# dernasherbrezon/sdr-server

Measured on AMD Instinct MI355X. Metric: input IQ Msamples/s processed (all clients), 2.016 Msps->48 kHz xlating FIR, higher is better.
Workload: dtype f32; 1 GPU; 1024 clients x 48 kHz off one 2.016 Msps cu8 stream, D=42, 505 taps, 262144-byte blocks (BASELINE configs[3]; N=1: the >=1000-client single-GPU target); clients_total=1024, clients_per_gpu=1024, blocks_per_call=8, mode=optimized, parallelism=single GPU, rccl_ranks=1, feed=xlating_multi (C host)

## Files before the change

sdr-server_amd/csrc/xl_dev_inline.h:

```cpp
#ifndef XL_DEV_INLINE_H_
#define XL_DEV_INLINE_H_
#include "xl_device.h"
#include "xl_q15_narrow.h"

typedef float v2f __attribute__((ext_vector_type(2)));
typedef float v4f __attribute__((ext_vector_type(4)));
typedef const float __attribute__((address_space(4))) *cfloat_p;
typedef const uint32_t __attribute__((address_space(4))) *cu32_p;

#define XL_DEV static __device__ __forceinline__
#define XL_MEM __device__ __forceinline__

XL_DEV v2f xl_sample(const void *__restrict__ p, int fmt, uint32_t i) {
  v2f r;
  if (fmt == XLF_CU8) {
    const uint32_t v = reinterpret_cast<const uint16_t *>(p)[i];
    r.x = ((float)(v & 0xFFu) - 127.5f) / 128.0f;
    r.y = ((float)(v >> 8) - 127.5f) / 128.0f;
  } else if (fmt == XLF_CS8) {
    const int32_t v = reinterpret_cast<const int16_t *>(p)[i];
    r.x = (float)((int32_t)(int8_t)(v & 0xFF)) / 128.0f;
    r.y = (float)(v >> 8) / 128.0f;
  } else if (fmt == XLF_CS16) {
    const int32_t v = reinterpret_cast<const int32_t *>(p)[i];
// ... 72 lines not shown
};

template <int MODE>
XL_DEV v2f xl_rotate(const v2f a, const v2f p) {
  v2f r;
  if (MODE == 0) {
    r.x = a.x * p.x - a.y * p.y;
    r.y = a.x * p.y + a.y * p.x;
  } else {
    r.x = __builtin_fmaf(-a.y, p.y, a.x * p.x);
    r.y = __builtin_fmaf(a.y, p.x, a.x * p.y);
  }
  return r;
}

XL_DEV void xl_nco_step(v2f &p, const v2f inc) {
  v2f t1, t2;
  asm volatile(
      "v_pk_mul_f32 %0, %2, %3 op_sel_hi:[1,0]\n\t"
      "v_pk_mul_f32 %1, %2, %3 op_sel:[0,1] op_sel_hi:[1,1]"
      : "=&v"(t1), "=&v"(t2)
      : "v"(p), "v"(inc));
  asm volatile("v_pk_add_f32 %0, %1, %2 op_sel:[0,1] op_sel_hi:[1,0] neg_lo:[0,1]" : "=v"(p) : "v"(t1), "v"(t2));
}

XL_DEV v2f xl_nco_next(const v2f p, const v2f inc) {
  v2f t1, t2, r;
  asm volatile(
      "v_pk_mul_f32 %0, %3, %4 op_sel_hi:[1,0]\n\t"
      "v_pk_mul_f32 %1, %3, %4 op_sel:[0,1] op_sel_hi:[1,1]\n\t"
      "v_pk_add_f32 %2, %0, %1 op_sel:[0,1] op_sel_hi:[1,0] neg_lo:[0,1]"
      : "=&v"(t1), "=&v"(t2), "=&v"(r)
      : "v"(p), "v"(inc));
  return r;
}

XL_DEV v2f xl_nco_next_fma(const v2f p, const v2f inc) {
  v2f t, r;
  asm volatile(
      "v_pk_mul_f32 %0, %2, %3 op_sel:[1,1] op_sel_hi:[1,0]\n\t"
      "v_pk_fma_f32 %1, %2, %3, %0 op_sel_hi:[0,1,1] neg_lo:[0,0,1]"
      : "=&v"(t), "=&v"(r)
      : "v"(p), "v"(inc));
  return r;
}
XL_DEV v2f xl_nco_next_any(const v2f p, const v2f inc, const uint32_t flags) {
  return (flags & XL_POS_FMA_STEP) ? xl_nco_next_fma(p, inc) : xl_nco_next(p, inc);
}

XL_DEV v2f xl_nco_role_step(const v2f p, const v2f inc, const uint32_t flags) {
  float a, b, c, d;
  if (flags & XL_POS_FMA_STEP) {
    asm volatile(
        "v_mul_f32 %0, %3, %5\n\t"
        "v_mul_f32 %1, %3, %4\n\t"
        "v_fma_f32 %0, %2, %4, -%0\n\t"
        "v_fma_f32 %1, %2, %5, %1"
        : "=&v"(a), "=&v"(b)
        : "v"(p.x), "v"(p.y), "v"(inc.x), "v"(inc.y));
    return (v2f){a, b};
  }
  asm volatile(
      "v_mul_f32 %0, %4, %6\n\t"
      "v_mul_f32 %1, %5, %7\n\t"
      "v_mul_f32 %2, %4, %7\n\t"
      "v_mul_f32 %3, %5, %6\n\t"
      "v_sub_f32 %0, %0, %1\n\t"
      "v_add_f32 %1, %3, %2"
      : "=&v"(a), "=&v"(b), "=&v"(c), "=&v"(d)
      : "v"(p.x), "v"(p.y), "v"(inc.x), "v"(inc.y));
  return (v2f){a, b};
}

XL_DEV v2f xl_nco_renorm(const v2f p) {
  const double mag2 = (double)p.x * (double)p.x + (double)p.y * (double)p.y;
  const float mag = (float)__dsqrt_rn(mag2);
  return (v2f){p.x / mag, p.y / mag};
}

template <bool PACKED>
XL_DEV void xl_nco_client_chain(const XlNcoClient k, const XlBnd bnd, const uint32_t kb, const uint32_t ke,
                                const float2 *state_src, float2 *state_dst, float2 *__restrict__ tab,
                                unsigned long long *stamp = nullptr) {
  v2f p = {state_src[k.slot].x, state_src[k.slot].y};
  if (stamp) {
    asm volatile("s_waitcnt vmcnt(0)" ::: "memory");
    stamp[0] = wall_clock64();
  }
  if (bnd.K == 0u) {
    state_dst[k.slot] = make_float2(p.x, p.y);
    return;
  }
  const v2f inc = {k.incr.x, k.incr.y};
  v2f *__restrict__ o = reinterpret_cast<v2f *>(tab) + (k.out_off >> XL_PH_SHIFT);
  v4f *__restrict__ o4 = reinterpret_cast<v4f *>(o);
  uint32_t m = kb;
  while (m < ke) {
    const uint32_t nb = xl_bnd_next(bnd, m);
    const uint32_t me = nb < ke ? nb : ke;
    for (; m < me && (m & (2u * XL_PH_STRIDE - 1u)) != 0u; ++m) {
      if (tab != nullptr && (m & (XL_PH_STRIDE - 1u)) == 0u) o[m >> XL_PH_SHIFT] = p;
      p = PACKED ? xl_nco_next_any(p, inc, bnd.flags) : xl_nco_role_step(p, inc, bnd.flags);
    }
    for (; !(bnd.flags & XL_POS_FMA_STEP) && m + 2u * XL_PH_STRIDE <= me; m += 2u * XL_PH_STRIDE) {
      const v2f q0 = p;
      for (uint32_t i = 0; i < XL_PH_STRIDE; i += 16u) {
#pragma unroll
        for (int j = 0; j < 16; ++j) p = PACKED ? xl_nco_next(p, inc) : xl_nco_role_step(p, inc, 0u);
      }
      const v2f q1 = p;
      for (uint32_t i = 0; i < XL_PH_STRIDE; i += 16u) {
#pragma unroll
        for (int j = 0; j < 16; ++j) p = PACKED ? xl_nco_next(p, inc) : xl_nco_role_step(p, inc, 0u);
      }
      if (tab != nullptr) o4[m >> (XL_PH_SHIFT + 1u)] = (v4f){q0.x, q0.y, q1.x, q1.y};
    }
    for (; m < me; ++m) {
      if (tab != nullptr && (m & (XL_PH_STRIDE - 1u)) == 0u) o[m >> XL_PH_SHIFT] = p;
      p = PACKED ? xl_nco_next_any(p, inc, bnd.flags) : xl_nco_role_step(p, inc, bnd.flags);
    }
    if (me == nb) p = xl_nco_renorm(p);
  }
  if (stamp) stamp[1] = wall_clock64();
  state_dst[k.slot] = make_float2(p.x, p.y);
}

XL_DEV XlBnd xl_nco_bnd(const XlNcoClient k, const XlPos pos, const uint32_t explicit_K) {
  XlBnd b;
  if (explicit_K != 0xFFFFFFFFu) {
    b.j0 = 0u, b.D = k.D, b.S = 0xFFFFFFFFu, b.G = 1u, b.K = explicit_K;
  } else {
    const XlDyn d = xl_grid_dyn(k.D, 1u, k.rem0, 0u, pos);
    b.j0 = d.j0, b.D = k.D, b.S = pos.S, b.G = pos.G, b.K = d.K;
  }
  b.flags = pos.pad;
  return b;
}

template <class Store>
XL_DEV void xl_phase_walk(v2f p, const uint32_t m0, const uint32_t count, const v2f inc, const XlBnd bnd, Store store) {
  uint32_t m = m0 & ~(XL_PH_STRIDE - 1u);
  uint32_t nb = xl_bnd_next(bnd, m);
  const uint32_t end = m0 + count;
  for (; m < end; ++m) {
    if (m >= m0) store(m - m0, p);
    p = xl_nco_next_any(p, inc, bnd.flags);
    if (m + 1u == nb) {
      p = xl_nco_renorm(p);
      nb = xl_bnd_next(bnd, m + 1u);
    }
  }
}

#endif
```

sdr-server_amd/csrc/xl_grid.h:

```cpp
#ifndef XL_GRID_H_
#define XL_GRID_H_
#include <stdint.h>

#define XL_HCAP 16384u
#define XL_PH_STRIDE 16u
#define XL_PH_SHIFT 4u

#if defined(__HIPCC__)
#define XL_HD __host__ __device__ static inline
#else
#define XL_HD static inline
#endif

typedef struct XlPos {
  uint32_t trel;
  uint32_t S;
  uint32_t G;
  uint32_t pad;
} XlPos;
#define XL_POS_NORENORM 1u
#define XL_POS_FMA_STEP 2u

typedef struct XlDyn {
  uint32_t base;
  uint32_t K;
  uint32_t zero_below;
  uint32_t j0;
} XlDyn;

XL_HD XlDyn xl_grid_dyn_cap(uint32_t D, uint32_t T, uint32_t rem0, uint32_t hv0, XlPos p, uint32_t hcap) {
  const uint32_t rem = (rem0 % D + p.trel % D) % D;
  const uint32_t j0 = (D - rem) % D;
  const uint32_t N = p.S * p.G;
  uint32_t hv = hv0 + (p.trel < hcap ? p.trel : hcap);
  XlDyn d;
  if (hv > hcap) hv = hcap;
  d.j0 = j0;
  d.K = N > j0 ? (N - j0 + D - 1u) / D : 0u;
  d.base = hcap - (T - 1u) + j0;
  d.zero_below = hcap - hv;
  return d;
}

XL_HD XlDyn xl_grid_dyn(uint32_t D, uint32_t T, uint32_t rem0, uint32_t hv0, XlPos p) {
  return xl_grid_dyn_cap(D, T, rem0, hv0, p, XL_HCAP);
}

XL_HD XlPos xl_grid_next(XlPos p) {
  XlPos n = p;
  n.trel = p.trel + p.S * p.G;
  return n;
}

XL_HD uint32_t xl_grid_mstart(uint32_t j0, uint32_t D, uint32_t S, uint32_t g) {
  const uint32_t n = g * S;
  return n > j0 ? (n - j0 + D - 1u) / D : 0u;
}

typedef struct XlBnd {
  uint32_t j0, D, S, G, K;
  uint32_t flags;
} XlBnd;

XL_HD uint32_t xl_bnd_next(const XlBnd b, uint32_t m) {
  uint32_t g, nb;
  if (b.flags & XL_POS_NORENORM) return 0xFFFFFFFFu;
  if (b.G <= 1u) return b.K;
  g = (b.j0 + m * b.D) / b.S;
  if (g + 1u >= b.G) return b.K;
  nb = xl_grid_mstart(b.j0, b.D, b.S, g + 1u);
  return nb < b.K ? nb : b.K;
}

XL_HD uint32_t xl_merge_j0(uint32_t j0_ref, uint32_t delta, uint32_t D) {
  const uint32_t j = j0_ref + delta;
  return j >= D ? j - D : j;
}
XL_HD uint32_t xl_merge_shift(uint32_t j0_ref, uint32_t delta, uint32_t D) { return j0_ref + delta >= D ? 0u : 1u; }
XL_HD uint32_t xl_merge_points(uint32_t D, XlPos p) { return (p.S * p.G + D - 1u) / D + 1u; }
XL_HD uint32_t xl_merge_outputs(uint32_t j0_ref, uint32_t delta, uint32_t D, XlPos p) {
  const uint32_t N = p.S * p.G, Ka = N / D;
  return Ka + (xl_merge_j0(j0_ref, delta, D) < N - Ka * D ? 1u : 0u);
}

typedef struct XlColDuty {
  XlBnd bnd;
  uint32_t shift;
  uint32_t ibeg;
  uint32_t m0;
  uint32_t ok;
  uint32_t tab;
} XlColDuty;
XL_HD XlColDuty xl_col_duty(uint32_t j0_ref, uint32_t delta, uint32_t D, XlPos p, uint32_t V, uint32_t s, uint32_t g, int vacant) {
  XlColDuty d;
  uint32_t q0;
  d.bnd.j0 = xl_merge_j0(j0_ref, delta, D), d.bnd.D = D, d.bnd.S = p.S, d.bnd.G = p.G, d.bnd.flags = p.pad;
  d.bnd.K = xl_merge_outputs(j0_ref, delta, D, p);
  d.shift = xl_merge_shift(j0_ref, delta, D);
  q0 = s * V + g * XL_PH_STRIDE;
  d.ibeg = q0 < d.shift ? 1u : 0u;
  d.m0 = q0 + d.ibeg - d.shift;
  d.ok = !vacant && g * XL_PH_STRIDE < V && d.m0 < d.bnd.K ? 1u : 0u;
  d.tab = d.ok ? d.m0 >> XL_PH_SHIFT : 0u;
  return d;
}
XL_HD uint32_t xl_col_duty_count(XlColDuty d) {
  const uint32_t left = d.bnd.K - d.m0, span = XL_PH_STRIDE - d.ibeg;
  return d.ok ? (left < span ? left : span) : 0u;
}

#endif
```

sdr-server_amd/csrc/xl_inv32.hip:

```cpp
#include "xl_poly_dev.h"

#include "xl_inv32_layout.h"

#include <hip/hip_ext.h>

typedef float v4f __attribute__((ext_vector_type(4)));
typedef uint32_t v4u __attribute__((ext_vector_type(4)));

#define XLI32_WPE 3
#define XLI32_WAVES 2
__global__ __launch_bounds__(64 * XLI32_WAVES) __attribute__((amdgpu_waves_per_eu(XLI32_WPE, XLI32_WPE))) void xlp_inverse32_kernel(const XlpArgs a) {
  constexpr uint32_t WAVES = XLI32_WAVES, M = 128u, CW = 32u, NSUB = XLP_COLS / CW;
  __shared__ __attribute__((aligned(16))) unsigned char region[WAVES][XLI32_WAVE_BYTES];
  uint32_t bid;
  if (!xlp_work_block(a, bid)) return;
  const uint32_t w = __builtin_amdgcn_readfirstlane(threadIdx.x >> 6), j = threadIdx.x & 63u;
  const uint32_t unit = bid * WAVES + w;
  const uint32_t half = unit & 1u, sub = (unit >> 1) % NSUB;
  const uint32_t qq = (unit >> 1) / NSUB;
  const uint32_t cg = qq % a.ncg, s = qq / a.ncg;
  if (s >= a.nseg) return;
  unsigned char *const reg = region[w];
  v2f tw0, tw1;
  {
    const v2f *__restrict__ W = reinterpret_cast<const v2f *>(a.W);
    tw0 = W[(2u * (j & 3u) * (j >> 2)) & 255u];
    tw1 = W[(2u * (j & 3u) * ((j >> 2) + 16u)) & 255u];
  }
  static_assert(XL_PH_STRIDE == 16u, "one table entry per lane and round: 8 entries per column and segment");
  const uint32_t col0 = cg * XLP_COLS + sub * CW + 16u * half;
  XlpCol ce[2];
#pragma unroll
  for (int r = 0; r < 2; ++r) ce[r] = a.cols[col0 + 8u * r + xli32_walk_c8(j)];
  v2f z[32];
  {
    const v2f *__restrict__ tile = reinterpret_cast<const v2f *>(a.Y) + xly_tile(a.nseg_cap, M, cg, s, sub);
    const uint32_t o0 = xli32_load(half, j, 0u);
#pragma unroll
    for (int m2 = 0; m2 < 32; ++m2) z[m2] = tile[o0 + m2 * 4u * CW];
  }
  {
    tw0.y = -tw0.y, tw1.y = -tw1.y;
    *reinterpret_cast<v2f *>(reg + xli32_tw(j >> 2, j & 3u)) = tw0 * (1.0f / (float)M);
    *reinterpret_cast<v2f *>(reg + xli32_tw((j >> 2) + 16u, j & 3u)) = tw1 * (1.0f / (float)M);
  }
  __builtin_amdgcn_wave_barrier();
  xl_fft32_inverse<v2f, XlpFftOps>(z);
#pragma unroll
  for (int i = 0; i < 32; ++i) asm volatile("" : "+v"(z[i]));
  const uint32_t gq = xli32_walk_gq(j);
  XlBnd ebnd[2];
  uint32_t m0[2], cnt[2];
  v2f pe[2];
#pragma unroll
  for (int r = 0; r < 2; ++r) {
    const XlColDuty du = xl_col_duty(a.j0_ref, ce[r].delta, a.D, a.pos, a.V, s, gq, ce[r].out_off == 0xFFFFFFFFu);
    ebnd[r] = du.bnd, cnt[r] = xl_col_duty_count(du);
    pe[r] = reinterpret_cast<const v2f *>(a.phtab)[du.ok ? (ce[r].out_off >> XL_PH_SHIFT) + du.tab : 0u];
    if (gq == 0u) *reinterpret_cast<v4u *>(reg + xli32_meta(8u * r + xli32_walk_c8(j))) = (v4u){ce[r].out_off, du.shift, ce[r].out_off != 0xFFFFFFFFu ? du.bnd.K : 0u, du.ibeg};
    m0[r] = du.m0 | du.ibeg << 31;
  }
  {
    const unsigned char *const twp = reg + xli32_tw(0u, xli32_load_m1(j));
#pragma unroll
    for (int t = 0; t < 32; ++t) z[xli32_slot32(t)] = xlp_cmul_v(z[xli32_slot32(t)], *reinterpret_cast<const v2f *>(twp + t * 32));
  }
  const uint32_t cc = xli32_cc(j), t = xli32_t(j);
  const uint32_t qs0 = s * a.V + t;
#pragma unroll
  for (int r = 0; r < 2; ++r) {
    if ((xli32_load_c(j) >> 3) == (uint32_t)r) {
      unsigned char *const wr = reg + xli32_exch(xli32_load_c(j) & 7u, xli32_load_m1(j), 0u);
#pragma unroll
      for (int i = 0; i < 16; ++i) {
        const v2f p0 = z[xli32_slot32(2 * i)], p1 = z[xli32_slot32(2 * i + 1)];
        *reinterpret_cast<v4f *>(wr + i * 16) = (v4f){p0.x, p0.y, p1.x, p1.y};
      }
    }
    __builtin_amdgcn_wave_barrier();
    v2f y[4][4];
    {
      const unsigned char *const rd = reg + xli32_exch(cc, 0u, t);
#pragma unroll
      for (int k = 0; k < 4; ++k)
#pragma unroll
        for (int m1 = 0; m1 < 4; ++m1) y[k][m1] = *reinterpret_cast<const v2f *>(rd + k * 2 * XLI32_XCOL + m1 * XLI32_XROW);
    }
    __builtin_amdgcn_wave_barrier();
#pragma unroll
    for (int k = 0; k < 4; ++k) xl_fft4_inverse<v2f, XlpFftOps>(y[k]);
    if (cnt[r] != 0u) {
      const uint32_t ibeg = m0[r] >> 31;
      unsigned char *const pw = reg + xli32_phase(xli32_walk_c8(j), gq * XL_PH_STRIDE + ibeg);
      xl_phase_walk(pe[r], m0[r] & 0x7FFFFFFFu, cnt[r], (v2f){ce[r].incr.x, ce[r].incr.y}, ebnd[r],
                    [&](uint32_t i, v2f phs) { *reinterpret_cast<v2f *>(pw + i * 8u) = phs; });
    }
    __builtin_amdgcn_wave_barrier();
    {
      const unsigned char *const pr = reg + xli32_phase(cc, t);
      const unsigned char *const mr = reg + xli32_meta(8u * r + cc);
#pragma unroll
      for (int k = 0; k < 4; ++k) {
        const v4u mt = *reinterpret_cast<const v4u *>(mr + k * 32);
        v2f *__restrict__ out = reinterpret_cast<v2f *>(a.out) + mt.x;
#pragma unroll
        for (int g = 0; g < 4; ++g) {
          const uint32_t qo = t + 32u * g, idx = qs0 + 32u * g - mt.y;
          if (qo < a.V && idx < mt.z)
            out[idx] = xl_rotate<1>(y[k][g], *reinterpret_cast<const v2f *>(pr + k * 2 * XLI32_PCOL + g * 2 * XLI32_PROW));
        }
      }
    }
    __builtin_amdgcn_wave_barrier();
  }
}

uint32_t xlp_inverse32_work(uint32_t tiles) { return (2u * tiles + XLI32_WAVES - 1u) / XLI32_WAVES; }

void xlp_inverse32_launch(const XlpArgs &a, const dim3 grid, hipStream_t s, hipEvent_t done) {
  if (done) hipExtLaunchKernelGGL(xlp_inverse32_kernel, grid, dim3(64u * XLI32_WAVES), 0, s, nullptr, done, 0, a);
  else hipLaunchKernelGGL(xlp_inverse32_kernel, grid, dim3(64u * XLI32_WAVES), 0, s, a);
}
```

sdr-server_amd/csrc/xl_inv8.hip:

```cpp
#include "xl_poly_dev.h"

#include "xl_inv8_layout.h"

#include <hip/hip_ext.h>

typedef float v4f __attribute__((ext_vector_type(4)));

__global__ __launch_bounds__(256) __attribute__((amdgpu_waves_per_eu(4, 4))) void xlp_inverse8_kernel(const XlpArgs a) {
  constexpr uint32_t M = 128u, CW = 32u, NSUB = XLP_COLS / CW;
  __shared__ __attribute__((aligned(16))) unsigned char region[4][XLI8_WAVE_BYTES];
  __shared__ v2f twl[16][8];
  uint32_t bid;
  if (!xlp_work_block(a, bid)) return;
  const uint32_t sub = bid % NSUB;
  const uint32_t q = bid / NSUB;
  const uint32_t cg = q % a.ncg, s = q / a.ncg;
  const uint32_t w = __builtin_amdgcn_readfirstlane(threadIdx.x >> 6), j = threadIdx.x & 63u;
  v2f z[16];
  {
    const v2f *__restrict__ tile = reinterpret_cast<const v2f *>(a.Y) + xly_tile(a.nseg_cap, M, cg, s, sub);
    const uint32_t o0 = xli8_load(w, j, 0u);
    constexpr uint32_t os = 8u * CW;
#pragma unroll
    for (int m2 = 0; m2 < 16; ++m2) z[m2] = tile[o0 + m2 * os];
  }
  if (threadIdx.x < 128u) {
    v2f tv = reinterpret_cast<const v2f *>(a.W)[(2u * (threadIdx.x & 7u) * (threadIdx.x >> 3)) & 255u];
    tv.y = -tv.y;
    twl[threadIdx.x >> 3][threadIdx.x & 7u] = tv;
  }
  static_assert(XL_PH_STRIDE == 16u, "one table entry per lane: 8 entries per column and segment");
  const uint32_t c8 = xli8_col(j), u = xli8_u(j);
  const XlpCol ce = a.cols[cg * XLP_COLS + sub * CW + 8u * w + c8];
  const XlColDuty du = xl_col_duty(a.j0_ref, ce.delta, a.D, a.pos, a.V, s, u, ce.out_off == 0xFFFFFFFFu);
  const v2f pe = reinterpret_cast<const v2f *>(a.phtab)[du.ok ? (ce.out_off >> XL_PH_SHIFT) + du.tab : 0u];
  __syncthreads();
  unsigned char *const reg = region[w];
  xl_fft16_inverse<v2f, XlpFftOps>(z);
  {
    const uint32_t m1 = xli8_load_m1(j);
    const v2f *__restrict__ twp = &twl[0][m1];
    unsigned char *const wr = reg + xli8_exch(xli8_load_c8(j), 0u, m1);
    *reinterpret_cast<v2f *>(wr) = z[xli8_slot16(0)];
#pragma unroll
    for (int t = 1; t < 16; ++t) *reinterpret_cast<v2f *>(wr + t * XLI8_XROW) = xlp_cmul_v(z[xli8_slot16(t)], twp[t * 8]);
  }
  __builtin_amdgcn_wave_barrier();
  v2f y[2][8];
  {
    const unsigned char *const rd = reg + xli8_exch(c8, u, 0u);
#pragma unroll
    for (int e = 0; e < 2; ++e)
#pragma unroll
      for (int i = 0; i < 4; ++i) {
        const v4f pr = *reinterpret_cast<const v4f *>(rd + e * 8 * XLI8_XROW + i * 16);
        y[e][2 * i] = (v2f){pr.x, pr.y};
        y[e][2 * i + 1] = (v2f){pr.z, pr.w};
      }
  }
  __builtin_amdgcn_wave_barrier();
  xl_fft8_inverse<v2f, XlpFftOps>(y[0]);
  xl_fft8_inverse<v2f, XlpFftOps>(y[1]);
  if (du.ok) {
    unsigned char *const pw = reg + xli8_phase(c8, u * XL_PH_STRIDE + du.ibeg);
    xl_phase_walk(pe, du.m0, xl_col_duty_count(du), (v2f){ce.incr.x, ce.incr.y}, du.bnd,
                  [&](uint32_t i, v2f phs) { *reinterpret_cast<v2f *>(pw + i * 8u) = phs; });
  }
  __builtin_amdgcn_wave_barrier();
  if (ce.out_off != 0xFFFFFFFFu) {
    v2f *__restrict__ out = reinterpret_cast<v2f *>(a.out) + ce.out_off;
    const unsigned char *const pr = reg + xli8_phase(c8, u);
    const uint32_t qs0 = s * a.V + u;
#pragma unroll
    for (int g = 0; g < 8; ++g)
#pragma unroll
      for (int e = 0; e < 2; ++e) {
        const uint32_t qo = 16u * g + 8u * e + u, qs = qs0 + 16u * g + 8u * e;
        if (qo < a.V && qs >= du.shift && qs - du.shift < du.bnd.K) {
          const v2f val = y[e][xli8_slot8(g)] * (1.0f / (float)M);
          out[qs - du.shift] = xl_rotate<1>(val, *reinterpret_cast<const v2f *>(pr + g * XLI8_PROW + e * 64));
        }
      }
  }
}

void xlp_inverse8_launch(const XlpArgs &a, const dim3 grid, hipStream_t s, hipEvent_t done) {
  if (done) hipExtLaunchKernelGGL(xlp_inverse8_kernel, grid, dim3(256), 0, s, nullptr, done, 0, a);
  else hipLaunchKernelGGL(xlp_inverse8_kernel, grid, dim3(256), 0, s, a);
}
```

sdr-server_amd/csrc/xl_polyphase.h:

```cpp
#ifndef XL_POLYPHASE_H_
#define XL_POLYPHASE_H_
#include "xl_device.h"
#include "xl_plan_rules.h"
#include "xl_y_layout.h"

#define XLP_M_MAX 256u
#define XLP_SEG 16u
#define XLP_XS 16u
#define XLP_COLS 128u
#define XLP_NKB_MAX 14u
#define XLP_NKB_4W 8u
#define XLP_H_XSCALE 128.0f
#define XLP_H_RMAX 8192.0f
#define XLP_SEGMAX_STRIDE 32u
#define XLP_FWD_GROUP_MIN_WGS 96u
#define XLP_BSTEP 2u

static inline bool xlp_ximg_eligible(uint32_t fmt, uint32_t mix_kind, uint32_t nkb, uint32_t M) {
  return fmt != XLF_CF32 && mix_kind == 1u && nkb >= 1u && nkb <= XLP_NKB_4W && (M == 128u || M == 256u);
}

static_assert(XLP_COLS == XLY_COLS, "a column group of the Y image (xl_y_layout.h) is a mix workgroup's columns");

struct XlpCol {
  uint32_t out_off;
  uint32_t delta;
  float2 incr;
};

struct XlpArgs {
  const void *in0;
  const void *in1;
  uint32_t n0, n1;
  uint32_t fmt;
  XlPos pos;
  uint32_t j0_ref;
  uint32_t base;
  uint32_t Kq;
  uint32_t zero_below;
  uint32_t D, Dpad;
  uint32_t T, A, V;
  uint32_t M;
  uint32_t mix_passes;
  uint32_t nseg;
  uint32_t nseg_cap;
  uint32_t ncg;
  uint32_t exp;
  uint32_t inv_reg;
  uint32_t mix_kind;
  uint32_t nkb;
  uint32_t mix_pp;
  uint32_t *segmax;
  uint32_t seg_par, seg_cap;
  unsigned long long *trace;
  const float2 *W;
  float2 *X;
  uint32_t ximg;
  const void *Rh;
  const float *cscale;
  float2 *Y;
  const XlpCol *cols;
  const float2 *phtab;
  float2 *out;
  void *hist_out;
  uint32_t hist_units, block_units, roll_blocks;
  const XlNcoClient *nco_clients;
  uint32_t nco_nclients;
  uint32_t nco_blocks;
  uint32_t nco_prio;
  uint32_t nco_skip_at, nco_skip;
  uint32_t nco_k0, nco_k1;
  const float2 *nco_state_src;
  float2 *nco_state_dst;
  float2 *nco_tab;
};

hipError_t xlp_launch_tables_h(const float2 *rt, const uint32_t *delta, const uint32_t *colidx, const float *scale,
                               uint32_t nlist, uint32_t T, uint32_t D, uint32_t A, uint32_t M, uint32_t nkb, void *Rh,
                               hipStream_t s);
static inline size_t xlp_rh_bytes_per_group(uint32_t M, uint32_t nkb) { return (size_t)M * 4u * 2u * nkb * 64u * 16u; }
hipError_t xlp_launch_tables_f(const float2 *rt, const uint32_t *delta, const uint32_t *colidx, uint32_t nlist, uint32_t T, uint32_t D,
                               uint32_t A, uint32_t M, uint32_t nb8, void *Rf, hipStream_t s);
hipError_t xlp_launch_mix_f32(const XlpArgs &a, hipStream_t s);
void xlp_mix_wide_launch(const XlpArgs &a, hipStream_t s);
hipError_t xlp_launch_forward(const XlpArgs &a, hipStream_t s);
hipError_t xlp_launch_mix(const XlpArgs &a, hipStream_t s);
hipError_t xlp_launch_inverse(const XlpArgs &a, hipStream_t s, hipEvent_t done);
void xlp_inverse8_launch(const XlpArgs &a, const dim3 grid, hipStream_t s, hipEvent_t done);
uint32_t xlp_inverse32_work(uint32_t tiles);
void xlp_inverse32_launch(const XlpArgs &a, const dim3 grid, hipStream_t s, hipEvent_t done);

#endif
```

sdr-server_amd/csrc/xl_polyphase.hip:

```cpp
#include "xl_polyphase.h"

#include "xl_poly_dev.h"
#include "xl_mix_layout.h"
#include "xl_xop_layout.h"

#include <hip/hip_ext.h>

typedef uint32_t xlp_u2 __attribute__((ext_vector_type(2)));
typedef uint32_t xlp_u4 __attribute__((ext_vector_type(4)));
typedef uint32_t xlp_u1_a2 __attribute__((aligned(2)));
typedef xlp_u2 xlp_u2_a2 __attribute__((aligned(2)));
typedef xlp_u2 xlp_u2_a4 __attribute__((aligned(4)));
typedef xlp_u4 xlp_u4_a4 __attribute__((aligned(4)));
typedef xlp_u4 xlp_u4_a8 __attribute__((aligned(8)));
template <int NB>
XL_DEV void xlp_samples(const void *__restrict__ p, const int fmt, const uint32_t i, v2f (&out)[NB]) {
  static_assert(NB == 1 || NB == 2 || NB == 4, "one, two or four adjacent samples");
  if (NB == 1) {
    out[0] = xl_sample(p, fmt, i);
    return;
  }
  uint32_t w[2 * NB];
  if (fmt == XLF_CU8 || fmt == XLF_CS8) {
    const char *q = reinterpret_cast<const char *>(p) + 2u * (size_t)i;
// ... 113 lines not shown
      }
    }
#pragma unroll
    for (int n = 0; n < NB; ++n) u[n][r] = v[n];
  }
  unsigned long long t_loaded = 0ull;
  if (a.trace) {
    __builtin_amdgcn_s_waitcnt(0);
    t_loaded = wall_clock64();
  }
#pragma unroll
  for (int c0 = 0; c0 < NB; c0 += NBD) {
    v2f *bufs[NBD];
    uint32_t rs0[NBD];
#pragma unroll
    for (int n = 0; n < NBD; ++n) bufs[n] = lds[h][n], rs0[n] = 0u;
    v2f *const(&cb)[NBD] = bufs;
    const uint32_t(&crs)[NBD] = rs0;
    xlp_dft<-1, NBD, M>(*reinterpret_cast<v2f(*)[NBD][4]>(&u[c0]), cb, tw, l, crs);
  }
  if (IMG) {
    uint32_t hp[2][NB][4];
#pragma unroll
    for (int n = 0; n < NB; ++n)
#pragma unroll
      for (int r = 0; r < 4; ++r) {
        _Float16 r1, r2, i1, i2;
        xlp_split_h(u[n][r].x * XLP_H_XSCALE, r1, r2);
        xlp_split_h(u[n][r].y * XLP_H_XSCALE, i1, i2);
        const bool real = b0 + (uint32_t)n < a.D;
        hp[0][n][r] = real ? xlp_pack_h(r1, i1) : 0u;
        hp[1][n][r] = real ? xlp_pack_h(r2, i2) : 0u;
      }
    uint4 *const stg = reinterpret_cast<uint4 *>(&lds[0][0][0]);
    uint4 *__restrict__ const img = reinterpret_cast<uint4 *>(a.X);
    constexpr int RC = M == 256 ? 2 : 4;
#pragma unroll
    for (int rc = 0; rc < 4; rc += RC) {
      __syncthreads();
#pragma unroll
      for (int term = 0; term < 2; ++term)
#pragma unroll
        for (int r = rc; r < rc + RC; ++r) {
          const uint32_t ml = l + L * (uint32_t)(r - rc);
          stg[((uint32_t)term * 128u + ml) * XOP_SEG + (h ^ (ml & 15u))] = (uint4){hp[term][0][r], hp[term][1][r], hp[term][2][r], hp[term][3][r]};
        }
      __syncthreads();
      for (uint32_t i = j; i < 2u * 128u * XOP_SEG; i += NT) {
        const uint32_t ml = (i >> 4) & 127u, term = i >> 11, sl = (i & 15u) ^ (ml & 15u);
        img[xop_bin_base(M, a.nkb, pass, ml + L * (uint32_t)rc) + xop_in_bin(a.nkb, term, grp, sl)] = stg[i];
      }
    }
    return;
  }
  if (a.segmax != nullptr) {
    float mx = 0.0f;
#pragma unroll
    for (int n = 0; n < NB; ++n)
      if (b0 + (uint32_t)n < a.D) {
#pragma unroll
        for (int r = 0; r < 4; ++r) mx = fmaxf(mx, fmaxf(fabsf(u[n][r].x), fabsf(u[n][r].y)));
      }
    atomicMax(&tmax(h), __float_as_uint(mx));
  }
#pragma unroll
  for (int n = 0; n < NBD; ++n)
#pragma unroll
    for (int r = 0; r < 4; ++r) lds[h][n][l + L * r] = u[n][r];
  __syncthreads();
  if (smax != nullptr && tmax(j) > seen) atomicMax(smax, tmax(j));
  if (a.segmax != nullptr && bid == 0u)
    for (uint32_t i = j; i < a.seg_cap; i += NT) a.segmax[((size_t)(a.seg_par ^ 1u) * a.seg_cap + i) * XLP_SEGMAX_STRIDE] = 0u;
  static_assert(XLP_XS == 16u && XLP_SEG <= XLP_XS, "image rows of 16 complex = 8 x 16 bytes");
  unsigned long long t_xf = 0ull;
#pragma unroll
  for (int n = 0; n < NBD; ++n) {
    if (b0 + (uint32_t)n >= a.D) break;
    v4f *__restrict__ X = reinterpret_cast<v4f *>(a.X) + ((size_t)pass * a.Dpad + b0 + (uint32_t)n) * M * (XLP_XS / 2u);
    for (uint32_t i = j; i < (uint32_t)M * (XLP_XS / 2u); i += NT) {
      const uint32_t m = i >> 3, part = i & 7u;
      const v2f x0 = 2u * part < XLP_SEG ? lds[2u * part][n][m] : (v2f){0.0f, 0.0f};
      const v2f x1 = 2u * part + 1u < XLP_SEG ? lds[2u * part + 1u][n][m] : (v2f){0.0f, 0.0f};
      X[i] = (v4f){x0.x, x0.y, x1.x, x1.y};
    }
  }
  if (a.trace && bid < 6000u) {
    t_xf = wall_clock64();
    __builtin_amdgcn_s_waitcnt(0);
    if (j == 0u) {
      unsigned long long *t = a.trace + 4096 + 4 * (size_t)bid;
      t[0] = t_begin;
      t[1] = wall_clock64();
      t[2] = t_loaded;
      t[3] = t_xf;
    }
  }
}

template <int M, class P>
XL_DEV void xlp_inverse_body(const XlpArgs &a) {
  constexpr bool SWZ = !__is_same(P, XlpPosPad);
  static_assert(!SWZ || M == 128, "the swizzled layout is written for rows of 128 elements");
  constexpr uint32_t L = M / 4;
  constexpr uint32_t CW = xly_tile_columns(M);
  constexpr uint32_t WPC = CW / 4;
  constexpr uint32_t NSUB = XLP_COLS / CW;
  __shared__ v2f tile[CW][SWZ ? M : XLP_ROW(M) - 1];
  if (xlp_work_role_or_skip(a)) return;
  const unsigned long long t_begin = a.trace ? wall_clock64() : 0ull;
  const uint32_t bid = xlp_work_index(a);
  const uint32_t sub = bid % NSUB;
  const uint32_t q = bid / NSUB;
  const uint32_t cg = q % a.ncg, s = q / a.ncg;
  const uint32_t w = __builtin_amdgcn_readfirstlane(threadIdx.x >> 6), j = threadIdx.x & 63u;
  const uint32_t h = j / L, l = j % L;
  const XlpTw tw = xlp_twiddles<+1, M>(reinterpret_cast<const v2f *>(a.W), l);
  {
    constexpr uint32_t PARTS = CW / 2, MR = 256 / PARTS;
    const uint32_t part = threadIdx.x % PARTS, mrow = threadIdx.x / PARTS;
    v4f v[8];
    {
      const v4f *__restrict__ src = reinterpret_cast<const v4f *>(a.Y + xly_tile(a.nseg_cap, M, cg, s, sub)) + part;
#pragma unroll
      for (int i = 0; i < 8; ++i) v[i] = src[(size_t)(mrow + MR * i) * PARTS];
    }
#pragma unroll
    for (int i = 0; i < 8; ++i) {
      const uint32_t m = mrow + MR * i;
      tile[2 * part][P::pos(m, XLP_SWZ_ROW(2u * part))] = (v2f){v[i].x, v[i].y};
      tile[2 * part + 1][P::pos(m, XLP_SWZ_ROW(2u * part + 1u))] = (v2f){v[i].z, v[i].w};
    }
  }
  constexpr uint32_t GQ = M / XL_PH_STRIDE;
  static_assert(WPC * GQ == 64u, "one expansion duty per lane");
  const v2f *__restrict__ ph = reinterpret_cast<const v2f *>(a.phtab);
  v2f *__restrict__ out = reinterpret_cast<v2f *>(a.out);
  const uint32_t colbase = cg * XLP_COLS + sub * CW + WPC * w;
  const uint32_t sV = s * a.V;
  uint32_t idx[4], rel[4], span[4];
#pragma unroll
  for (int n = 0; n < 4; ++n) {
    const XlpCol c = a.cols[colbase + 4u * h + n];
    const uint32_t ksh = xl_merge_shift(a.j0_ref, c.delta, a.D);
    const uint32_t end = ksh + xl_merge_outputs(a.j0_ref, c.delta, a.D, a.pos);
    const uint32_t lo = ksh > sV ? ksh - sV : 0u;
    const uint32_t left = end > sV ? end - sV : 0u;
    const uint32_t hi = c.out_off == 0xFFFFFFFFu ? 0u : (left < a.V ? left : a.V);
    idx[n] = c.out_off + sV + l + 1u - ksh;
    rel[n] = l - lo;
    span[n] = hi > lo ? hi - lo : 0u;
  }
  const uint32_t en = j / GQ, gq = j % GQ;
  const XlpCol ce = a.cols[colbase + en];
  const XlColDuty du = xl_col_duty(a.j0_ref, ce.delta, a.D, a.pos, a.V, s, gq, ce.out_off == 0xFFFFFFFFu);
  const v2f pe = ph[du.ok ? (ce.out_off >> XL_PH_SHIFT) + du.tab : 0u];
  __syncthreads();
  const unsigned long long t_loaded = a.trace ? wall_clock64() : 0ull;
  v2f u[4][4];
  v2f *const rows[4] = {tile[WPC * w + 4u * h], tile[WPC * w + 4u * h + 1], tile[WPC * w + 4u * h + 2],
                        tile[WPC * w + 4u * h + 3]};
  const uint32_t rbase = WPC * w + 4u * h;
  const uint32_t rs[4] = {XLP_SWZ_ROW(rbase), XLP_SWZ_ROW(rbase + 1u), XLP_SWZ_ROW(rbase + 2u), XLP_SWZ_ROW(rbase + 3u)};
#pragma unroll
  for (int n = 0; n < 4; ++n)
#pragma unroll
    for (int r = 0; r < 4; ++r) u[n][r] = rows[n][P::pos(l + L * r, rs[n])];
  __builtin_amdgcn_wave_barrier();
  xlp_dft<+1, 4, M, P>(u, rows, tw, l, rs);
  __builtin_amdgcn_wave_barrier();
  if (du.ok) {
    v2f *__restrict__ row = tile[WPC * w + en];
    const uint32_t ers = XLP_SWZ_ROW(WPC * w + en);
    const uint32_t p0 = gq * XL_PH_STRIDE + du.ibeg;
    xl_phase_walk(pe, du.m0, xl_col_duty_count(du), (v2f){ce.incr.x, ce.incr.y}, du.bnd,
                  [&](uint32_t i, v2f phs) { row[P::pos(p0 + i, ers)] = phs; });
  }
  __builtin_amdgcn_wave_barrier();
  const unsigned long long t_xf = a.trace ? wall_clock64() : 0ull;
  v2f phs[4][4];
#pragma unroll
  for (int n = 0; n < 4; ++n)
#pragma unroll
    for (int r = 0; r < 4; ++r) phs[n][r] = rows[n][P::pos(l + L * r, rs[n])];
#pragma unroll
  for (int n = 0; n < 4; ++n) {
    asm volatile("" : "+v"(idx[n]));
    v2f *__restrict__ const po = out - 1 + idx[n];
#pragma unroll
    for (int r = 0; r < 4; ++r) {
      const v2f y = u[n][r] * (1.0f / (float)M);
      v2f z = xl_rotate<1>(y, phs[n][r]);
      asm volatile("" : "+v"(z));
      if (rel[n] + L * r < span[n]) po[L * r] = z;
    }
  }
  if (a.trace && threadIdx.x == 0 && bid < 6000u) {
    unsigned long long *t = a.trace + 4096 + 4 * (size_t)bid;
    t[0] = t_begin;
    t[1] = wall_clock64();
    t[2] = t_loaded;
    t[3] = t_xf;
  }
}

template <int M, class P = XlpPosPad>
__global__ __launch_bounds__(256) void xlp_inverse_kernel(const XlpArgs a) {
  xlp_inverse_body<M, P>(a);
}
__global__ __launch_bounds__(XLP_COLS) void xlp_tables_h_kernel(const float2 *__restrict__ rt,
                                                                const uint32_t *__restrict__ delta,
                                                                const uint32_t *__restrict__ colidx,
                                                                const float *__restrict__ scale, uint32_t nlist, uint32_t T,
                                                                uint32_t D, uint32_t A, uint32_t M, uint32_t nkb,
                                                                uint32_t *__restrict__ Rh) {
  __shared__ double wc[256], ws[256];
  for (uint32_t n = threadIdx.x; n < M; n += blockDim.x) sincospi(2.0 * (double)n / (double)M, &ws[n], &wc[n]);
  __syncthreads();
  const uint32_t m = blockIdx.x % M;
  const uint32_t b = blockIdx.x / M;
  const uint32_t j = blockIdx.y * XLP_COLS + threadIdx.x;
  if (j >= nlist) return;
  const uint32_t col = colidx[j];
  double sr, si;
  xlp_branch_spectrum(rt, nlist, j, delta[j], T, D, A, M, m, b, wc, ws, sr, si);
  const float sc = scale[j];
  _Float16 r1, r2, i1, i2;
  xlp_split_h((float)sr * sc, r1, r2);
  xlp_split_h(-(float)si * sc, i1, i2);
  const uint32_t cg = col / XLP_COLS, cl = col % XLP_COLS;
  const uint32_t w = cl >> 5, ln = xlm_lane(xlm_half(b), cl & 31u);
  Rh[xlm_rh_slot(cg, M, m, w, 0u, nkb, xlm_kblock(b), ln) * 4u + xlm_dword(b)] = xlp_pack_h(r1, i1);
  Rh[xlm_rh_slot(cg, M, m, w, 1u, nkb, xlm_kblock(b), ln) * 4u + xlm_dword(b)] = xlp_pack_h(r2, i2);
}

static bool xlp_valid_m(uint32_t M) { return M == 64u || M == 128u || M == 256u; }

hipError_t xlp_launch_tables_h(const float2 *rt, const uint32_t *delta, const uint32_t *colidx, const float *scale,
                               uint32_t nlist, uint32_t T, uint32_t D, uint32_t A, uint32_t M, uint32_t nkb, void *Rh,
                               hipStream_t s) {
  if (!xlp_valid_m(M) || nlist == 0u || nkb == 0u || nkb > XLP_NKB_MAX || D > 8u * nkb) return hipErrorInvalidValue;
  hipLaunchKernelGGL(xlp_tables_h_kernel, dim3(M * 8u * nkb, (nlist + XLP_COLS - 1u) / XLP_COLS), dim3(XLP_COLS), 0, s, rt, delta,
                     colidx, scale, nlist, T, D, A, M, nkb, reinterpret_cast<uint32_t *>(Rh));
  return hipGetLastError();
}

hipError_t xlp_launch_forward(const XlpArgs &a, hipStream_t s) {
  if (!xlp_valid_m(a.M)) return hipErrorInvalidValue;
  const uint32_t passes = (a.nseg + XLP_SEG - 1u) / XLP_SEG;
  const uint32_t nb = a.M == 256u ? 2u : 4u;
  const uint32_t ngrp = (a.D + nb - 1u) / nb;
  const bool grouped = a.fmt == XLF_CF32 && passes * ngrp >= XLP_FWD_GROUP_MIN_WGS;
  if (a.ximg) {
    if (!xlp_ximg_eligible(a.fmt, a.mix_kind, a.nkb, a.M) || a.D > 8u * a.nkb || a.segmax != nullptr) return hipErrorInvalidValue;
    const dim3 gridi(a.nco_blocks + passes * ((a.D + XOP_GROUP - 1u) / XOP_GROUP) + a.roll_blocks);
    if (a.M == 256u) hipLaunchKernelGGL((xlp_forward_kernel<256, 4, true>), gridi, dim3(XLP_SEG * 64u), 0, s, a);
    else hipLaunchKernelGGL((xlp_forward_kernel<128, 4, true>), gridi, dim3(XLP_SEG * 32u), 0, s, a);
    return hipGetLastError();
  }
  const dim3 grid(a.nco_blocks + passes * (grouped ? ngrp : a.D) + a.roll_blocks);
  if (a.M == 256u) {
    if (grouped) hipLaunchKernelGGL((xlp_forward_kernel<256, 2>), grid, dim3(XLP_SEG * 64u), 0, s, a);
    else hipLaunchKernelGGL((xlp_forward_kernel<256, 1>), grid, dim3(XLP_SEG * 64u), 0, s, a);
  } else if (a.M == 64u) {
    if (grouped) hipLaunchKernelGGL((xlp_forward_kernel<64, 4>), grid, dim3(XLP_SEG * 16u), 0, s, a);
    else hipLaunchKernelGGL((xlp_forward_kernel<64, 1>), grid, dim3(XLP_SEG * 16u), 0, s, a);
  } else {
    if (grouped) hipLaunchKernelGGL((xlp_forward_kernel<128, 4>), grid, dim3(XLP_SEG * 32u), 0, s, a);
    else hipLaunchKernelGGL((xlp_forward_kernel<128, 1>), grid, dim3(XLP_SEG * 32u), 0, s, a);
  }
  return hipGetLastError();
}

static XlpArgs xlp_checked_skip(const XlpArgs &a, uint32_t work_blocks) {
  XlpArgs b = a;
  if (b.nco_skip == 0u || b.nco_skip_at < b.nco_blocks || b.nco_skip_at + b.nco_skip > b.nco_blocks + work_blocks) {
    b.nco_skip = 0u;
    b.nco_skip_at = 0xFFFFFFFFu;
  }
  return b;
}

hipError_t xlp_launch_inverse(const XlpArgs &a0, hipStream_t s, hipEvent_t done) {
  if (!xlp_valid_m(a0.M)) return hipErrorInvalidValue;
  const uint32_t tiles = a0.nseg * a0.ncg * (XLP_COLS / xly_tile_columns(a0.M));
  const uint32_t kind = xlp_inverse_pick(a0.M, a0.inv_reg, tiles);
  const uint32_t work = kind == 6u ? xlp_inverse32_work(tiles) : tiles;
  const XlpArgs a = xlp_checked_skip(a0, work);
  const dim3 grid(a.nco_blocks + a.nco_skip + work);
  if (kind == 6u) {
    xlp_inverse32_launch(a, grid, s, done);
    return hipGetLastError();
  }
  if (kind == 5u) {
    xlp_inverse8_launch(a, grid, s, done);
    return hipGetLastError();
  }
  void (*kern)(const XlpArgs) = a.M == 256u ? xlp_inverse_kernel<256, XlpPosPad>
                                : (a.M == 64u ? xlp_inverse_kernel<64, XlpPosPad> : xlp_inverse_kernel<128, XlpPosSwz>);
  if (done) hipExtLaunchKernelGGL(kern, grid, dim3(256), 0, s, nullptr, done, 0, a);
  else hipLaunchKernelGGL(kern, grid, dim3(256), 0, s, a);
  return hipGetLastError();
}
```

Before: 5.803 million Msamples/s.

## Expand per-column phase tables on a fixed lane grid with a uniform unrolled NCO path

Replaces the per-column duty computation, which gave each lane a variable start and count for its phase walk, with a grid-aligned duty: every lane expands a full XL_PH_STRIDE block of phases (plus extra entries on the last group) from its table entry and stores only those inside the valid span. A fully unrolled, wave-uniform NCO loop is used unless a wave-level ballot finds a renormalisation boundary inside the range, in which case it falls back to the general walk. Renorm boundaries are located with host-precomputed 32-bit reciprocals of S and D instead of integer division. The intent is to remove divergence and serial loop overhead in the phase-expansion step of the inverse FFT kernels, at the cost of computing some phases that are never stored and recomputing the duty after the FFT to save registers.

```diff
diff --git a/sdr-server_amd/csrc/xl_dev_inline.h b/sdr-server_amd/csrc/xl_dev_inline.h
--- a/sdr-server_amd/csrc/xl_dev_inline.h
+++ b/sdr-server_amd/csrc/xl_dev_inline.h
@@ -248,4 +248,38 @@
   }
 }
 
+XL_DEV XlGridDuty xl_grid_duty_again(const uint32_t j0_ref, uint32_t delta, uint32_t out_off, const uint32_t D, const XlPos pos,
+                                     const uint32_t V, const uint32_t s, const uint32_t g) {
+  asm volatile("" : "+v"(delta), "+v"(out_off));
+  return xl_grid_duty(j0_ref, delta, D, pos, V, s, g, out_off == 0xFFFFFFFFu);
+}
+
+template <class Store>
+XL_DEV void xl_phase_expand(v2f p, const XlGridDuty du, const bool last, const uint32_t extra, const v2f inc, const uint32_t rS,
+                            const uint32_t rD, Store store) {
+  if (__builtin_amdgcn_ballot_w64(du.span != 0u) == 0ull) return;
+  const uint32_t n = XL_PH_STRIDE + (last ? extra : 0u);
+  const uint32_t iend = du.span - du.rel < n ? du.span - du.rel : n;
+  bool slow = (du.bnd.flags & XL_POS_FMA_STEP) != 0u;
+  if (!slow && !(du.bnd.flags & XL_POS_NORENORM) && du.bnd.G > 1u) {
+    const uint32_t nb = xl_bnd_next_rcp(du.bnd, rS, rD, du.ma);
+    slow = __builtin_amdgcn_ballot_w64(du.span != 0u && nb - du.ma < iend) != 0ull;
+  }
+  if (!slow) {
+    if (du.rel < du.span) store(0u, p);
+#pragma unroll
+    for (uint32_t i = 1u; i < XL_PH_STRIDE; ++i) {
+      p = xl_nco_next(p, inc);
+      if (du.rel + i < du.span) store(i, p);
+    }
+    for (uint32_t e = 0u; e < extra; ++e) {
+      p = xl_nco_next(p, inc);
+      if (last && du.rel + XL_PH_STRIDE + e < du.span) store(XL_PH_STRIDE + e, p);
+    }
+  } else if (du.span != 0u) {
+    const uint32_t i0 = (int32_t)du.rel < 0 ? 0u - du.rel : 0u;
+    xl_phase_walk(p, du.ma + i0, iend - i0, inc, du.bnd, [&](uint32_t i, v2f phs) { store(i0 + i, phs); });
+  }
+}
+
 #endif
diff --git a/sdr-server_amd/csrc/xl_grid.h b/sdr-server_amd/csrc/xl_grid.h
--- a/sdr-server_amd/csrc/xl_grid.h
+++ b/sdr-server_amd/csrc/xl_grid.h
@@ -109,4 +109,49 @@
   return d.ok ? (left < span ? left : span) : 0u;
 }
 
+XL_HD uint32_t xl_grid_extra(uint32_t M, uint32_t V) { return V + (XL_PH_STRIDE - 1u) > M ? V + (XL_PH_STRIDE - 1u) - M : 0u; }
+
+typedef struct XlGridDuty {
+  XlBnd bnd;
+  uint32_t shift;
+  uint32_t ma;
+  uint32_t pos;
+  uint32_t rel;
+  uint32_t span;
+  uint32_t tab;
+} XlGridDuty;
+XL_HD XlGridDuty xl_grid_duty(uint32_t j0_ref, uint32_t delta, uint32_t D, XlPos p, uint32_t V, uint32_t s, uint32_t g, int vacant) {
+  XlGridDuty d;
+  uint32_t qlo, qhi, m_lo, m_hi;
+  d.bnd.j0 = xl_merge_j0(j0_ref, delta, D), d.bnd.D = D, d.bnd.S = p.S, d.bnd.G = p.G, d.bnd.flags = p.pad;
+  d.bnd.K = xl_merge_outputs(j0_ref, delta, D, p);
+  d.shift = xl_merge_shift(j0_ref, delta, D);
+  qlo = s * V > d.shift ? s * V : d.shift;
+  qhi = s * V + V < d.shift + d.bnd.K ? s * V + V : d.shift + d.bnd.K;
+  m_lo = qlo - d.shift;
+  m_hi = qhi > qlo ? qhi - d.shift : m_lo;
+  d.ma = (m_lo & ~(XL_PH_STRIDE - 1u)) + g * XL_PH_STRIDE;
+  d.pos = d.ma + d.shift - s * V;
+  d.rel = d.ma - m_lo;
+  d.span = !vacant && d.ma < m_hi ? m_hi - m_lo : 0u;
+  d.tab = d.span ? d.ma >> XL_PH_SHIFT : 0u;
+  return d;
+}
+
+XL_HD uint32_t xl_rcp32(uint32_t d) { return d > 1u ? (uint32_t)(0x100000000ull / d) : 0xFFFFFFFFu; }
+XL_HD uint32_t xl_div_rcp(uint32_t x, uint32_t d, uint32_t rcp) {
+  const uint32_t q = (uint32_t)(((uint64_t)x * rcp) >> 32);
+  return q + (x - q * d >= d ? 1u : 0u);
+}
+XL_HD uint32_t xl_bnd_next_rcp(const XlBnd b, uint32_t rS, uint32_t rD, uint32_t m) {
+  uint32_t g, n, nb;
+  if (b.flags & XL_POS_NORENORM) return 0xFFFFFFFFu;
+  if (b.G <= 1u) return b.K;
+  g = xl_div_rcp(b.j0 + m * b.D, b.S, rS);
+  if (g + 1u >= b.G) return b.K;
+  n = (g + 1u) * b.S;
+  nb = n > b.j0 ? xl_div_rcp(n - b.j0 + b.D - 1u, b.D, rD) : 0u;
+  return nb < b.K ? nb : b.K;
+}
+
 #endif
diff --git a/sdr-server_amd/csrc/xl_inv32.hip b/sdr-server_amd/csrc/xl_inv32.hip
--- a/sdr-server_amd/csrc/xl_inv32.hip
+++ b/sdr-server_amd/csrc/xl_inv32.hip
@@ -49,16 +49,12 @@
 #pragma unroll
   for (int i = 0; i < 32; ++i) asm volatile("" : "+v"(z[i]));
   const uint32_t gq = xli32_walk_gq(j);
-  XlBnd ebnd[2];
-  uint32_t m0[2], cnt[2];
   v2f pe[2];
 #pragma unroll
   for (int r = 0; r < 2; ++r) {
-    const XlColDuty du = xl_col_duty(a.j0_ref, ce[r].delta, a.D, a.pos, a.V, s, gq, ce[r].out_off == 0xFFFFFFFFu);
-    ebnd[r] = du.bnd, cnt[r] = xl_col_duty_count(du);
-    pe[r] = reinterpret_cast<const v2f *>(a.phtab)[du.ok ? (ce[r].out_off >> XL_PH_SHIFT) + du.tab : 0u];
-    if (gq == 0u) *reinterpret_cast<v4u *>(reg + xli32_meta(8u * r + xli32_walk_c8(j))) = (v4u){ce[r].out_off, du.shift, ce[r].out_off != 0xFFFFFFFFu ? du.bnd.K : 0u, du.ibeg};
-    m0[r] = du.m0 | du.ibeg << 31;
+    const XlGridDuty du = xl_grid_duty(a.j0_ref, ce[r].delta, a.D, a.pos, a.V, s, gq, ce[r].out_off == 0xFFFFFFFFu);
+    pe[r] = reinterpret_cast<const v2f *>(a.phtab)[du.span ? (ce[r].out_off >> XL_PH_SHIFT) + du.tab : 0u];
+    if (gq == 0u) *reinterpret_cast<v4u *>(reg + xli32_meta(8u * r + xli32_walk_c8(j))) = (v4u){ce[r].out_off, du.shift, ce[r].out_off != 0xFFFFFFFFu ? du.bnd.K : 0u, 0u};
   }
   {
     const unsigned char *const twp = reg + xli32_tw(0u, xli32_load_m1(j));
@@ -89,12 +85,9 @@
     __builtin_amdgcn_wave_barrier();
 #pragma unroll
     for (int k = 0; k < 4; ++k) xl_fft4_inverse<v2f, XlpFftOps>(y[k]);
-    if (cnt[r] != 0u) {
-      const uint32_t ibeg = m0[r] >> 31;
-      unsigned char *const pw = reg + xli32_phase(xli32_walk_c8(j), gq * XL_PH_STRIDE + ibeg);
-      xl_phase_walk(pe[r], m0[r] & 0x7FFFFFFFu, cnt[r], (v2f){ce[r].incr.x, ce[r].incr.y}, ebnd[r],
-                    [&](uint32_t i, v2f phs) { *reinterpret_cast<v2f *>(pw + i * 8u) = phs; });
-    }
+    const XlGridDuty du = xl_grid_duty_again(a.j0_ref, ce[r].delta, ce[r].out_off, a.D, a.pos, a.V, s, gq);
+    xl_phase_expand(pe[r], du, gq == 7u, xl_grid_extra(M, a.V), (v2f){ce[r].incr.x, ce[r].incr.y}, a.rcp_S, a.rcp_D,
+                    [&](uint32_t i, v2f phs) { *reinterpret_cast<v2f *>(reg + xli32_phase(xli32_walk_c8(j), du.pos + i)) = phs; });
     __builtin_amdgcn_wave_barrier();
     {
       const unsigned char *const pr = reg + xli32_phase(cc, t);
diff --git a/sdr-server_amd/csrc/xl_inv8.hip b/sdr-server_amd/csrc/xl_inv8.hip
--- a/sdr-server_amd/csrc/xl_inv8.hip
+++ b/sdr-server_amd/csrc/xl_inv8.hip
@@ -32,8 +32,8 @@
   static_assert(XL_PH_STRIDE == 16u, "one table entry per lane: 8 entries per column and segment");
   const uint32_t c8 = xli8_col(j), u = xli8_u(j);
   const XlpCol ce = a.cols[cg * XLP_COLS + sub * CW + 8u * w + c8];
-  const XlColDuty du = xl_col_duty(a.j0_ref, ce.delta, a.D, a.pos, a.V, s, u, ce.out_off == 0xFFFFFFFFu);
-  const v2f pe = reinterpret_cast<const v2f *>(a.phtab)[du.ok ? (ce.out_off >> XL_PH_SHIFT) + du.tab : 0u];
+  const XlGridDuty du = xl_grid_duty(a.j0_ref, ce.delta, a.D, a.pos, a.V, s, u, ce.out_off == 0xFFFFFFFFu);
+  const v2f pe = reinterpret_cast<const v2f *>(a.phtab)[du.span ? (ce.out_off >> XL_PH_SHIFT) + du.tab : 0u];
   __syncthreads();
   unsigned char *const reg = region[w];
   xl_fft16_inverse<v2f, XlpFftOps>(z);
@@ -61,11 +61,8 @@
   __builtin_amdgcn_wave_barrier();
   xl_fft8_inverse<v2f, XlpFftOps>(y[0]);
   xl_fft8_inverse<v2f, XlpFftOps>(y[1]);
-  if (du.ok) {
-    unsigned char *const pw = reg + xli8_phase(c8, u * XL_PH_STRIDE + du.ibeg);
-    xl_phase_walk(pe, du.m0, xl_col_duty_count(du), (v2f){ce.incr.x, ce.incr.y}, du.bnd,
-                  [&](uint32_t i, v2f phs) { *reinterpret_cast<v2f *>(pw + i * 8u) = phs; });
-  }
+  xl_phase_expand(pe, du, u == 7u, xl_grid_extra(M, a.V), (v2f){ce.incr.x, ce.incr.y}, a.rcp_S, a.rcp_D,
+                  [&](uint32_t i, v2f phs) { *reinterpret_cast<v2f *>(reg + xli8_phase(c8, du.pos + i)) = phs; });
   __builtin_amdgcn_wave_barrier();
   if (ce.out_off != 0xFFFFFFFFu) {
     v2f *__restrict__ out = reinterpret_cast<v2f *>(a.out) + ce.out_off;
diff --git a/sdr-server_amd/csrc/xl_polyphase.h b/sdr-server_amd/csrc/xl_polyphase.h
--- a/sdr-server_amd/csrc/xl_polyphase.h
+++ b/sdr-server_amd/csrc/xl_polyphase.h
@@ -34,6 +34,7 @@
   uint32_t n0, n1;
   uint32_t fmt;
   XlPos pos;
+  uint32_t rcp_S, rcp_D;
   uint32_t j0_ref;
   uint32_t base;
   uint32_t Kq;
diff --git a/sdr-server_amd/csrc/xl_polyphase.hip b/sdr-server_amd/csrc/xl_polyphase.hip
--- a/sdr-server_amd/csrc/xl_polyphase.hip
+++ b/sdr-server_amd/csrc/xl_polyphase.hip
@@ -289,8 +289,11 @@
   }
   const uint32_t en = j / GQ, gq = j % GQ;
   const XlpCol ce = a.cols[colbase + en];
-  const XlColDuty du = xl_col_duty(a.j0_ref, ce.delta, a.D, a.pos, a.V, s, gq, ce.out_off == 0xFFFFFFFFu);
-  const v2f pe = ph[du.ok ? (ce.out_off >> XL_PH_SHIFT) + du.tab : 0u];
+  v2f pe;
+  {
+    const XlGridDuty du = xl_grid_duty(a.j0_ref, ce.delta, a.D, a.pos, a.V, s, gq, ce.out_off == 0xFFFFFFFFu);
+    pe = ph[du.span ? (ce.out_off >> XL_PH_SHIFT) + du.tab : 0u];
+  }
   __syncthreads();
   const unsigned long long t_loaded = a.trace ? wall_clock64() : 0ull;
   v2f u[4][4];
@@ -305,12 +308,12 @@
   __builtin_amdgcn_wave_barrier();
   xlp_dft<+1, 4, M, P>(u, rows, tw, l, rs);
   __builtin_amdgcn_wave_barrier();
-  if (du.ok) {
+  {
     v2f *__restrict__ row = tile[WPC * w + en];
     const uint32_t ers = XLP_SWZ_ROW(WPC * w + en);
-    const uint32_t p0 = gq * XL_PH_STRIDE + du.ibeg;
-    xl_phase_walk(pe, du.m0, xl_col_duty_count(du), (v2f){ce.incr.x, ce.incr.y}, du.bnd,
-                  [&](uint32_t i, v2f phs) { row[P::pos(p0 + i, ers)] = phs; });
+    const XlGridDuty du = xl_grid_duty_again(a.j0_ref, ce.delta, ce.out_off, a.D, a.pos, a.V, s, gq);
+    xl_phase_expand(pe, du, gq == GQ - 1u, xl_grid_extra(M, a.V), (v2f){ce.incr.x, ce.incr.y}, a.rcp_S, a.rcp_D,
+                    [&](uint32_t i, v2f phs) { row[P::pos(du.pos + i, ers)] = phs; });
   }
   __builtin_amdgcn_wave_barrier();
   const unsigned long long t_xf = a.trace ? wall_clock64() : 0ull;
@@ -422,7 +425,8 @@
   const uint32_t tiles = a0.nseg * a0.ncg * (XLP_COLS / xly_tile_columns(a0.M));
   const uint32_t kind = xlp_inverse_pick(a0.M, a0.inv_reg, tiles);
   const uint32_t work = kind == 6u ? xlp_inverse32_work(tiles) : tiles;
-  const XlpArgs a = xlp_checked_skip(a0, work);
+  XlpArgs a = xlp_checked_skip(a0, work);
+  a.rcp_S = xl_rcp32(a.pos.S), a.rcp_D = xl_rcp32(a.D);
   const dim3 grid(a.nco_blocks + a.nco_skip + work);
   if (kind == 6u) {
     xlp_inverse32_launch(a, grid, s, done);
```

After: 5.900 million Msamples/s (median of 6 runs). 1.7% higher.
